# supranational/sppark

Hardware: NVIDIA H100
Metric: BLS12-381 G1 MSM/s @2^26 points (higher is better)
Workload: dtype u32x12 (384-bit Montgomery integers)

## Files before the change

### sppark_b200/build.py

```python
import os
import subprocess
import sys

HERE = os.path.dirname(os.path.abspath(__file__))
CSRC = os.path.join(HERE, "csrc")
LIB = os.environ.get("SPPARK_B200_LIB") or os.path.join(HERE, "libsppark_b200.so")

SOURCES = ["api.cu", "util/gpu.cu", "ntt/ntt.cu", "ntt/ntt_warp.cu", "poly/poly.cu", "msm/msm.cu", "msm/msm_bls12_381.cu", "msm/msm_bls12_381_g2.cu",
           "msm/msm_pasta.cu", "msm/msm_bn254_bls12_377.cu", "msm/msm_bn254_g2.cu", "msm/msm_bls12_377_g2.cu"]
NVCC_FLAGS = ["-std=c++17", "-O3", "-DSPPARK_B200_NO_WIDE_MSUB", "-gencode", "arch=compute_90a,code=sm_90a", "-lineinfo",
              "-Xcompiler", "-fPIC", "--threads", "4"]


def _sources():
    return [os.path.join(CSRC, s) for s in SOURCES if os.path.exists(os.path.join(CSRC, s))]


def _newest_input():
    newest = 0.0
    for root, _, files in os.walk(CSRC):
        for f in files:
            newest = max(newest, os.path.getmtime(os.path.join(root, f)))
    inc = os.path.join(os.path.dirname(HERE), "include", "sppark_b200.h")
    return max(newest, os.path.getmtime(inc))


def _up_to_date(obj, flags):
    dep = obj[:-2] + ".d"
    try:
        if open(obj + ".flags").read() != " ".join(flags):
            return False
        t = os.path.getmtime(obj)
        words = open(dep).read().replace("\\\n", " ").split()
        return all(os.path.getmtime(w) <= t for w in words[1:] if not w.endswith(":"))
    except OSError:
        return False


def build(force=False, verbose=False):
    if not force and os.path.exists(LIB) and os.path.getmtime(LIB) >= _newest_input():
        return LIB
    objs = []
    procs = []
    extra = os.environ.get("SPPARK_B200_NVCC_EXTRA", "").split()
    objdir = os.path.join(HERE, "build" + ("_" + os.path.basename(LIB) if extra else ""))
    os.makedirs(objdir, exist_ok=True)
    for src in _sources():
        obj = os.path.join(objdir, os.path.basename(src).replace(".cu", ".o"))
        objs.append(obj)
        if not force and not verbose and _up_to_date(obj, [*NVCC_FLAGS, *extra]):
            continue
        cmd = ["nvcc", *NVCC_FLAGS, *extra, "-MD", "-c", "-o", obj, src]
        if verbose:
            cmd.insert(1, "-Xptxas=-v")
        with open(obj + ".flags", "w") as f:
            f.write(" ".join([*NVCC_FLAGS, *extra]))
        procs.append((subprocess.Popen(cmd), cmd))
    for p, cmd in procs:
        if p.wait() != 0:
            raise RuntimeError("nvcc failed: " + " ".join(cmd))
    subprocess.check_call(["nvcc", "-shared", "-o", LIB, *objs, "-gencode", "arch=compute_90a,code=sm_90a"])
    return LIB


if __name__ == "__main__":
    print(build(force="--force" in sys.argv, verbose="-v" in sys.argv))
```

### sppark_b200/csrc/ec/xyzz.cuh

```cuda
#pragma once
#include "../ff/mont.cuh"

namespace ec {

template<class F> struct affine_t {
    F X, Y;
    HD bool is_inf() const
    {
        uint32_t acc = 0;
#pragma unroll
        for (int i = 0; i < F::N; i++) acc |= X.l[i] | Y.l[i];
        return acc == 0;
    }
};

template<class F> struct jacobian_t {
    F X, Y, Z;
};

template<class F> struct xyzz_t {
    F X, Y, ZZZ, ZZ;

    HD void set_inf()
    {
        X = F::zero(); Y = F::zero(); ZZZ = F::zero(); ZZ = F::zero();
    }
    HD bool is_inf() const
    {
        uint32_t acc = 0;
#pragma unroll
        for (int i = 0; i < F::N; i++) acc |= ZZZ.l[i] | ZZ.l[i];
        return acc == 0;
    }
    HD void set_affine(const affine_t<F>& p)
    {
        X = p.X; Y = p.Y; ZZZ = F::one(); ZZ = F::one();
    }

    HD_NOINLINE void set_double_of(const affine_t<F>& p)
    {
        F U = p.Y.dbl();
        F V = U.sqr();
        F W = U * V;
        F S = p.X * V;
        F M = p.X.sqr();
        M = M.dbl() + M;
        F X3 = M.sqr() - S - S;
        Y = M * (S - X3) - W * p.Y;
        X = X3;
        ZZ = V;
        ZZZ = W;
    }

    HD void madd(const affine_t<F>& p2)
    {
        if (p2.is_inf()) return;
        if (is_inf()) { set_affine(p2); return; }
        F P = F::mul_shared(p2.X, ZZ) - X;
        F R = F::mul_shared(p2.Y, ZZZ) - Y;
        if (P.is_zero()) {
            if (R.is_zero()) set_double_of(p2);
            else set_inf();
            return;
        }
        F PP = F::sqr_shared(P);
        F PPP = F::mul_shared(P, PP);
        F Q = F::mul_shared(X, PP);
        F X3 = F::sqr_shared(R) - PPP - Q - Q;
        Y = F::msub_shared(R, Q - X3, Y, PPP);
        X = X3;
        ZZ = F::mul_shared(ZZ, PP);
        ZZZ = F::mul_shared(ZZZ, PPP);
    }

    HD_NOINLINE void dbl()
    {
        if (is_inf()) return;
        F U = Y.dbl();
        F V = U.sqr();
        F W = U * V;
        F S = X * V;
        F M = X.sqr();
        M = M.dbl() + M;
        F X3 = M.sqr() - S - S;
        Y = M * (S - X3) - W * Y;
        X = X3;
        ZZ = ZZ * V;
        ZZZ = ZZZ * W;
    }

    HD_NOINLINE void add(const xyzz_t& p2)
    {
        if (p2.is_inf()) return;
        if (is_inf()) { *this = p2; return; }
        F U1 = X * p2.ZZ;
        F S1 = Y * p2.ZZZ;
        F P = p2.X * ZZ - U1;
        F R = p2.Y * ZZZ - S1;
        if (P.is_zero()) {
            if (R.is_zero()) dbl();
            else set_inf();
            return;
        }
        F PP = P.sqr();
        F PPP = P * PP;
        F Q = U1 * PP;
        F X3 = R.sqr() - PPP - Q - Q;
        Y = R * (Q - X3) - S1 * PPP;
        X = X3;
        ZZ = ZZ * p2.ZZ * PP;
        ZZZ = ZZZ * p2.ZZZ * PPP;
    }


    HD void dbl_hot()
    {
        if (is_inf()) return;
        F U = Y.dbl();
        F V = F::mul_shared(U, U);
        F W = F::mul_shared(U, V);
        F S = F::mul_shared(X, V);
        F M = F::mul_shared(X, X);
        M = M.dbl() + M;
        F X3 = F::mul_shared(M, M) - S - S;
        Y = F::mul_shared(M, S - X3) - F::mul_shared(W, Y);
        X = X3;
        ZZ = F::mul_shared(ZZ, V);
        ZZZ = F::mul_shared(ZZZ, W);
    }
    HD void add_hot(const xyzz_t& p2)
    {
        if (p2.is_inf()) return;
        if (is_inf()) { *this = p2; return; }
        F U1 = F::mul_shared(X, p2.ZZ);
        F S1 = F::mul_shared(Y, p2.ZZZ);
        F P = F::mul_shared(p2.X, ZZ) - U1;
        F R = F::mul_shared(p2.Y, ZZZ) - S1;
        if (P.is_zero()) {
            if (R.is_zero()) dbl_hot();
            else set_inf();
            return;
        }
        F PP = F::mul_shared(P, P);
        F PPP = F::mul_shared(P, PP);
        F Q = F::mul_shared(U1, PP);
        F X3 = F::mul_shared(R, R) - PPP - Q - Q;
        Y = F::mul_shared(R, Q - X3) - F::mul_shared(S1, PPP);
        X = X3;
        ZZ = F::mul_shared(F::mul_shared(ZZ, p2.ZZ), PP);
        ZZZ = F::mul_shared(F::mul_shared(ZZZ, p2.ZZZ), PPP);
    }

    HD jacobian_t<F> to_jacobian() const
    {
        jacobian_t<F> r;
        if (is_inf()) { r.X = F::zero(); r.Y = F::zero(); r.Z = F::zero(); return r; }
        r.X = X * ZZ;
        r.Y = Y * ZZZ;
        r.Z = ZZ;
        return r;
    }
};

}
```

### sppark_b200/csrc/ff/mont.cuh

```cuda
#pragma once
#include "../util/hd.cuh"

namespace ff {

#if defined(__CUDA_ARCH__)
namespace ptx {
DEV void mad_lo_cc(uint32_t& d, uint32_t a, uint32_t b, uint32_t c)
{   asm volatile("mad.lo.cc.u32 %0, %1, %2, %3;" : "=r"(d) : "r"(a), "r"(b), "r"(c));   }
DEV void madc_lo_cc(uint32_t& d, uint32_t a, uint32_t b, uint32_t c)
{   asm volatile("madc.lo.cc.u32 %0, %1, %2, %3;" : "=r"(d) : "r"(a), "r"(b), "r"(c));   }
DEV void madc_hi_cc(uint32_t& d, uint32_t a, uint32_t b, uint32_t c)
{   asm volatile("madc.hi.cc.u32 %0, %1, %2, %3;" : "=r"(d) : "r"(a), "r"(b), "r"(c));   }
DEV void addc(uint32_t& d, uint32_t a, uint32_t b)
{   asm volatile("addc.u32 %0, %1, %2;" : "=r"(d) : "r"(a), "r"(b));   }
DEV void add_cc(uint32_t& d, uint32_t a, uint32_t b)
{   asm volatile("add.cc.u32 %0, %1, %2;" : "=r"(d) : "r"(a), "r"(b));   }
DEV void addc_cc(uint32_t& d, uint32_t a, uint32_t b)
{   asm volatile("addc.cc.u32 %0, %1, %2;" : "=r"(d) : "r"(a), "r"(b));   }
DEV void sub_cc(uint32_t& d, uint32_t a, uint32_t b)
{   asm volatile("sub.cc.u32 %0, %1, %2;" : "=r"(d) : "r"(a), "r"(b));   }
DEV void subc_cc(uint32_t& d, uint32_t a, uint32_t b)
{   asm volatile("subc.cc.u32 %0, %1, %2;" : "=r"(d) : "r"(a), "r"(b));   }
DEV void subc(uint32_t& d, uint32_t a, uint32_t b)
{   asm volatile("subc.u32 %0, %1, %2;" : "=r"(d) : "r"(a), "r"(b));   }
}
#endif

template<class C>
struct mont_t {
    static constexpr int N = C::N;
    uint32_t l[N];

    static HD mont_t zero()
    {
        mont_t r;
#pragma unroll
        for (int i = 0; i < N; i++) r.l[i] = 0;
        return r;
    }
    static HD mont_t one()
    {
        mont_t r;
#pragma unroll
        for (int i = 0; i < N; i++) r.l[i] = C::ONE(i);
        return r;
    }
    static HD mont_t rr()
    {
        mont_t r;
#pragma unroll
        for (int i = 0; i < N; i++) r.l[i] = C::RR(i);
        return r;
    }
    HD bool is_zero() const
    {
        uint32_t acc = 0;
#pragma unroll
        for (int i = 0; i < N; i++) acc |= l[i];
        return acc == 0;
    }
    friend HD bool operator==(const mont_t& a, const mont_t& b)
    {
        uint32_t acc = 0;
#pragma unroll
        for (int i = 0; i < N; i++) acc |= a.l[i] ^ b.l[i];
        return acc == 0;
    }

    static HD mont_t final_sub(const mont_t& a, uint32_t top_carry = 0)
    {
        mont_t r;
#if defined(__CUDA_ARCH__)
        uint32_t t[N], borrow;
        ptx::sub_cc(t[0], a.l[0], C::P(0));
#pragma unroll
        for (int i = 1; i < N; i++) ptx::subc_cc(t[i], a.l[i], C::P(i));
        ptx::subc(borrow, top_carry, 0);
#pragma unroll
        for (int i = 0; i < N; i++) r.l[i] = borrow ? a.l[i] : t[i];
#else
        uint32_t t[N];
        int64_t br = 0;
        for (int i = 0; i < N; i++) {
            int64_t d = (int64_t)a.l[i] - C::P(i) + br;
            t[i] = (uint32_t)d;
            br = d >> 32;
        }
        br += top_carry;
        for (int i = 0; i < N; i++) r.l[i] = br < 0 ? a.l[i] : t[i];
#endif
        return r;
    }

    friend HD mont_t operator+(const mont_t& a, const mont_t& b)
    {
        mont_t s;
        uint32_t carry;
#if defined(__CUDA_ARCH__)
        ptx::add_cc(s.l[0], a.l[0], b.l[0]);
#pragma unroll
        for (int i = 1; i < N; i++) ptx::addc_cc(s.l[i], a.l[i], b.l[i]);
        ptx::addc(carry, 0, 0);
#else
        uint64_t c = 0;
        for (int i = 0; i < N; i++) {
            c += (uint64_t)a.l[i] + b.l[i];
            s.l[i] = (uint32_t)c;
            c >>= 32;
        }
        carry = (uint32_t)c;
#endif
        return final_sub(s, carry);
    }

    friend HD mont_t operator-(const mont_t& a, const mont_t& b)
    {
        mont_t d;
#if defined(__CUDA_ARCH__)
        uint32_t borrow;
        ptx::sub_cc(d.l[0], a.l[0], b.l[0]);
#pragma unroll
        for (int i = 1; i < N; i++) ptx::subc_cc(d.l[i], a.l[i], b.l[i]);
        ptx::subc(borrow, 0, 0);
        ptx::add_cc(d.l[0], d.l[0], C::P(0) & borrow);
#pragma unroll
        for (int i = 1; i < N - 1; i++) ptx::addc_cc(d.l[i], d.l[i], C::P(i) & borrow);
        ptx::addc(d.l[N - 1], d.l[N - 1], C::P(N - 1) & borrow);
#else
        int64_t br = 0;
        for (int i = 0; i < N; i++) {
            int64_t x = (int64_t)a.l[i] - b.l[i] + br;
            d.l[i] = (uint32_t)x;
            br = x >> 32;
        }
        if (br) {
            uint64_t c = 0;
            for (int i = 0; i < N; i++) {
                c += (uint64_t)d.l[i] + C::P(i);
                d.l[i] = (uint32_t)c;
                c >>= 32;
            }
        }
#endif
        return d;
    }

    HD mont_t neg() const { return is_zero() ? *this : zero() - *this; }
    HD mont_t cneg(bool flag) const { return flag ? neg() : *this; }
    HD mont_t dbl() const { return *this + *this; }

#if defined(__CUDA_ARCH__)
    template<int I, class V>
    static DEV void row(uint32_t (&E)[2 * N + 2], uint32_t (&O)[2 * N + 2], uint32_t x, const V& v)
    {
        constexpr bool even_row = (I & 1) == 0;
        uint32_t (&A1)[2 * N + 2] = even_row ? E : O;
        uint32_t (&A2)[2 * N + 2] = even_row ? O : E;
        ptx::mad_lo_cc(A1[I], x, v[0], A1[I]);
        ptx::madc_hi_cc(A1[I + 1], x, v[0], A1[I + 1]);
#pragma unroll
        for (int j = 2; j < N; j += 2) {
            ptx::madc_lo_cc(A1[I + j], x, v[j], A1[I + j]);
            ptx::madc_hi_cc(A1[I + j + 1], x, v[j], A1[I + j + 1]);
        }
        ptx::addc(A1[I + N], A1[I + N], 0);
        ptx::mad_lo_cc(A2[I + 1], x, v[1], A2[I + 1]);
        ptx::madc_hi_cc(A2[I + 2], x, v[1], A2[I + 2]);
#pragma unroll
        for (int j = 3; j < N; j += 2) {
            ptx::madc_lo_cc(A2[I + j], x, v[j], A2[I + j]);
            ptx::madc_hi_cc(A2[I + j + 1], x, v[j], A2[I + j + 1]);
        }
        ptx::addc(A2[I + N + 1], A2[I + N + 1], 0);
    }

    struct modulus_view {
        DEV uint32_t operator[](int j) const { return C::P(j); }
    };

    template<int I>
    static DEV void rows(uint32_t (&E)[2 * N + 2], uint32_t (&O)[2 * N + 2], uint32_t& c,
                         const mont_t& a, const mont_t& b)
    {
        if constexpr (I < N) {
            row<I>(E, O, a.l[I], b.l);
            uint32_t m = (E[I] + O[I] + c) * C::M0;
            row<I>(E, O, m, modulus_view());
            uint64_t s = (uint64_t)E[I] + O[I] + c;
            c = (uint32_t)(s >> 32);
            rows<I + 1>(E, O, c, a, b);
        }
    }
#endif

    friend HD mont_t operator*(const mont_t& a, const mont_t& b) { return mul_inline(a, b); }

#if defined(__CUDA_ARCH__)
    struct wide_t { uint32_t l[2 * N]; };

    template<int I, int W, class V>
    static DEV void row_w(uint32_t* E, uint32_t* O, uint32_t x, const V& v)
    {
        uint32_t* A1 = (I & 1) == 0 ? E : O;
        uint32_t* A2 = (I & 1) == 0 ? O : E;
        ptx::mad_lo_cc(A1[I], x, v[0], A1[I]);
        ptx::madc_hi_cc(A1[I + 1], x, v[0], A1[I + 1]);
#pragma unroll
        for (int j = 2; j < W; j += 2) {
            ptx::madc_lo_cc(A1[I + j], x, v[j], A1[I + j]);
            ptx::madc_hi_cc(A1[I + j + 1], x, v[j], A1[I + j + 1]);
        }
        ptx::addc(A1[I + W + (W & 1)], A1[I + W + (W & 1)], 0);
        ptx::mad_lo_cc(A2[I + 1], x, v[1], A2[I + 1]);
        ptx::madc_hi_cc(A2[I + 2], x, v[1], A2[I + 2]);
#pragma unroll
        for (int j = 3; j < W; j += 2) {
            ptx::madc_lo_cc(A2[I + j], x, v[j], A2[I + j]);
            ptx::madc_hi_cc(A2[I + j + 1], x, v[j], A2[I + j + 1]);
        }
        ptx::addc(A2[I + W + 1 - (W & 1)], A2[I + W + 1 - (W & 1)], 0);
    }
    template<int I, int W>
    static DEV void mul_rows_w(uint32_t* E, uint32_t* O, const uint32_t* a, const uint32_t* b)
    {
        if constexpr (I < W) {
            row_w<I, W>(E, O, a[I], b);
            mul_rows_w<I + 1, W>(E, O, a, b);
        }
    }
    template<int W>
    static DEV void mul_wide_w(uint32_t* t, const uint32_t* a, const uint32_t* b)
    {
        uint32_t E[2 * W + 2], O[2 * W + 2];
#pragma unroll
        for (int i = 0; i < 2 * W + 2; i++) E[i] = O[i] = 0;
        mul_rows_w<0, W>(E, O, a, b);
        ptx::add_cc(t[0], E[0], O[0]);
#pragma unroll
        for (int i = 1; i < 2 * W - 1; i++) ptx::addc_cc(t[i], E[i], O[i]);
        ptx::addc(t[2 * W - 1], E[2 * W - 1], O[2 * W - 1]);
    }

    template<int W>
    static DEV uint32_t abs_diff_w(uint32_t* d, const uint32_t* x, const uint32_t* y)
    {
        uint32_t borrow;
        ptx::sub_cc(d[0], x[0], y[0]);
#pragma unroll
        for (int i = 1; i < W; i++) ptx::subc_cc(d[i], x[i], y[i]);
        ptx::subc(borrow, 0, 0);
        ptx::sub_cc(d[0], d[0] ^ borrow, borrow);
#pragma unroll
        for (int i = 1; i < W - 1; i++) ptx::subc_cc(d[i], d[i] ^ borrow, borrow);
        ptx::subc(d[W - 1], d[W - 1] ^ borrow, borrow);
        return borrow & 1;
    }

    static DEV wide_t mul_wide(const mont_t& a, const mont_t& b)
    {
        wide_t t;
#if defined(SPPARK_B200_KARATSUBA)
        constexpr bool karatsuba = N % 4 == 0 && N >= 8;
#else
        constexpr bool karatsuba = false;
#endif
        if constexpr (karatsuba) {
            constexpr int H = N / 2;
            uint32_t da[H], db[H], zm[2 * H], z0h[H], top, cf;
            const uint32_t neg = 0u - (abs_diff_w<H>(da, a.l, a.l + H) ^ abs_diff_w<H>(db, b.l + H, b.l));
            mul_wide_w<H>(t.l, a.l, b.l);
            mul_wide_w<H>(t.l + 2 * H, a.l + H, b.l + H);
            mul_wide_w<H>(zm, da, db);
#pragma unroll
            for (int i = 0; i < H; i++) z0h[i] = t.l[H + i];
            ptx::add_cc(t.l[H], t.l[H], t.l[2 * H]);
#pragma unroll
            for (int i = 1; i < 2 * H; i++) ptx::addc_cc(t.l[H + i], t.l[H + i], t.l[2 * H + i]);
            ptx::addc(top, 0, 0);
            ptx::add_cc(t.l[H], t.l[H], t.l[0]);
#pragma unroll
            for (int i = 1; i < H; i++) ptx::addc_cc(t.l[H + i], t.l[H + i], t.l[i]);
#pragma unroll
            for (int i = 0; i < H; i++) ptx::addc_cc(t.l[2 * H + i], t.l[2 * H + i], z0h[i]);
            ptx::addc(top, top, 0);
            ptx::add_cc(cf, neg, neg);
#pragma unroll
            for (int i = 0; i < 2 * H; i++) ptx::addc_cc(t.l[H + i], t.l[H + i], zm[i] ^ neg);
            ptx::addc(top, top, neg);
            ptx::add_cc(t.l[3 * H], t.l[3 * H], top);
#pragma unroll
            for (int i = 3 * H + 1; i < 2 * N - 1; i++) ptx::addc_cc(t.l[i], t.l[i], 0);
            ptx::addc(t.l[2 * N - 1], t.l[2 * N - 1], 0);
        } else {
            mul_wide_w<N>(t.l, a.l, b.l);
        }
        return t;
    }

    template<int I>
    static DEV void sqr_rows(uint32_t* E, uint32_t* O, uint32_t& c, const uint32_t* a, const uint32_t* d)
    {
        if constexpr (I < N) {
            if constexpr (I < N - 1) {
                uint32_t v[N - I];
                v[0] = a[I];
                v[1] = a[I + 1] << 1;
#pragma unroll
                for (int k = 2; k < N - I; k++) v[k] = d[I + k];
                row_w<2 * I, N - I>(E, O, a[I], v);
            } else {
                ptx::mad_lo_cc(E[2 * I], a[I], a[I], E[2 * I]);
                ptx::madc_hi_cc(E[2 * I + 1], a[I], a[I], E[2 * I + 1]);
                ptx::addc(E[2 * I + 2], E[2 * I + 2], 0);
            }
            uint32_t m = (E[I] + O[I] + c) * C::M0;
            row_w<I, N>(E, O, m, modulus_view());
            uint64_t s = (uint64_t)E[I] + O[I] + c;
            c = (uint32_t)(s >> 32);
            sqr_rows<I + 1>(E, O, c, a, d);
        }
    }
    static DEV mont_t sqr_inline(const mont_t& a)
    {
        if constexpr (C::P(N - 1) >= 0x55555555u) {
            return mul_inline(a, a);
        } else {
            uint32_t E[2 * N + 2], O[2 * N + 2], d[N], c = 0;
#pragma unroll
            for (int i = 0; i < 2 * N + 2; i++) E[i] = O[i] = 0;
#pragma unroll
            for (int j = 1; j < N; j++) d[j] = __funnelshift_l(a.l[j - 1], a.l[j], 1);
            sqr_rows<0>(E, O, c, a.l, d);
            mont_t r;
            ptx::add_cc(r.l[0], E[N], c);
#pragma unroll
            for (int i = 1; i < N; i++) ptx::addc_cc(r.l[i], E[N + i], 0);
            ptx::add_cc(r.l[0], r.l[0], O[N]);
#pragma unroll
            for (int i = 1; i < N - 1; i++) ptx::addc_cc(r.l[i], r.l[i], O[N + i]);
            ptx::addc(r.l[N - 1], r.l[N - 1], O[2 * N - 1]);
            return final_sub(r);
        }
    }

    static DEV wide_t sub_wide(const wide_t& x, const wide_t& y)
    {
        wide_t t;
        ptx::sub_cc(t.l[0], x.l[0], y.l[0]);
#pragma unroll
        for (int i = 1; i < 2 * N - 1; i++) ptx::subc_cc(t.l[i], x.l[i], y.l[i]);
        ptx::subc(t.l[2 * N - 1], x.l[2 * N - 1], y.l[2 * N - 1]);
        ptx::add_cc(t.l[N], t.l[N], C::P(0));
#pragma unroll
        for (int i = 1; i < N - 1; i++) ptx::addc_cc(t.l[N + i], t.l[N + i], C::P(i));
        ptx::addc(t.l[2 * N - 1], t.l[2 * N - 1], C::P(N - 1));
        return t;
    }

    template<int I>
    static DEV void redc_rows(uint32_t* E, uint32_t* O, uint32_t& c, const wide_t& t)
    {
        if constexpr (I < N) {
            uint32_t m = (t.l[I] + E[I] + O[I] + c) * C::M0;
            row_w<I, N>(E, O, m, modulus_view());
            uint64_t s = (uint64_t)t.l[I] + E[I] + O[I] + c;
            c = (uint32_t)(s >> 32);
            redc_rows<I + 1>(E, O, c, t);
        }
    }
    template<int K>
    static DEV mont_t redc(const wide_t& t)
    {
        uint32_t E[2 * N + 2], O[2 * N + 2], c = 0;
#pragma unroll
        for (int i = 0; i < 2 * N + 2; i++) E[i] = O[i] = 0;
        redc_rows<0>(E, O, c, t);
        mont_t r;
        uint32_t top, k;
        ptx::add_cc(r.l[0], t.l[N], c);
#pragma unroll
        for (int i = 1; i < N; i++) ptx::addc_cc(r.l[i], t.l[N + i], 0);
        ptx::addc(top, 0, 0);
        ptx::add_cc(r.l[0], r.l[0], E[N]);
#pragma unroll
        for (int i = 1; i < N; i++) ptx::addc_cc(r.l[i], r.l[i], E[N + i]);
        ptx::addc(k, 0, 0);
        top += k;
        ptx::add_cc(r.l[0], r.l[0], O[N]);
#pragma unroll
        for (int i = 1; i < N; i++) ptx::addc_cc(r.l[i], r.l[i], O[N + i]);
        ptx::addc(k, 0, 0);
        top += k;
        r = final_sub(r, top);
        if constexpr (K > 1) r = final_sub(r);
        return r;
    }

    static __device__ __noinline__ mont_t mul_shared(mont_t a, mont_t b)
    {
#if defined(SPPARK_B200_KARATSUBA)
        return redc<1>(mul_wide(a, b));
#else
        return mul_inline(a, b);
#endif
    }
    static __device__ __noinline__ mont_t sqr_shared(mont_t a) { return sqr_inline(a); }
    static __device__ __noinline__ mont_t msub_shared(mont_t a, mont_t b, mont_t c, mont_t d)
    {
#if defined(SPPARK_B200_NO_WIDE_MSUB)
        return mul_inline(a, b) - mul_inline(c, d);
#else
        return redc<2>(sub_wide(mul_wide(a, b), mul_wide(c, d)));
#endif
    }
#else
    static inline mont_t mul_shared(const mont_t& a, const mont_t& b) { return mul_inline(a, b); }
    static inline mont_t sqr_shared(const mont_t& a) { return mul_inline(a, a); }
    static inline mont_t msub_shared(const mont_t& a, const mont_t& b, const mont_t& c, const mont_t& d)
    {   return mul_inline(a, b) - mul_inline(c, d);   }
#endif

    static HD mont_t mul_inline(const mont_t& a, const mont_t& b)
    {
        mont_t r;
#if defined(__CUDA_ARCH__)
        uint32_t E[2 * N + 2], O[2 * N + 2], c = 0;
#pragma unroll
        for (int i = 0; i < 2 * N + 2; i++) E[i] = O[i] = 0;
        rows<0>(E, O, c, a, b);
        ptx::add_cc(r.l[0], E[N], c);
#pragma unroll
        for (int i = 1; i < N; i++) ptx::addc_cc(r.l[i], E[N + i], 0);
        ptx::add_cc(r.l[0], r.l[0], O[N]);
#pragma unroll
        for (int i = 1; i < N - 1; i++) ptx::addc_cc(r.l[i], r.l[i], O[N + i]);
        ptx::addc(r.l[N - 1], r.l[N - 1], O[2 * N - 1]);
#else
        uint32_t t[N + 2];
        for (int i = 0; i < N + 2; i++) t[i] = 0;
        for (int i = 0; i < N; i++) {
            uint64_t c = 0;
            for (int j = 0; j < N; j++) {
                c += (uint64_t)a.l[j] * b.l[i] + t[j];
                t[j] = (uint32_t)c;
                c >>= 32;
            }
            c += t[N];
            t[N] = (uint32_t)c;
            t[N + 1] = (uint32_t)(c >> 32);
            uint32_t m = t[0] * C::M0;
            c = ((uint64_t)m * C::P(0) + t[0]) >> 32;
            for (int j = 1; j < N; j++) {
                c += (uint64_t)m * C::P(j) + t[j];
                t[j - 1] = (uint32_t)c;
                c >>= 32;
            }
            c += t[N];
            t[N - 1] = (uint32_t)c;
            t[N] = t[N + 1] + (uint32_t)(c >> 32);
        }
        for (int i = 0; i < N; i++) r.l[i] = t[i];
        return final_sub(r, t[N]);
#endif
        return final_sub(r);
    }

    HD mont_t sqr() const { return *this * *this; }

    HD mont_t to_mont() const { return *this * rr(); }
    HD mont_t from_mont() const
    {
        mont_t o = zero();
        o.l[0] = 1;
        return *this * o;
    }
    HD mont_t inv() const
    {
        mont_t acc = one(), base = *this;
        uint32_t e[N];
        uint32_t borrow = 2;
        for (int i = 0; i < N; i++) {
            uint32_t pi = C::P(i);
            e[i] = pi - borrow;
            borrow = pi < borrow ? 1 : 0;
        }
        for (int i = N * 32 - 1; i >= 0; i--) {
            acc = acc.sqr();
            if ((e[i / 32] >> (i % 32)) & 1) acc = acc * base;
        }
        return acc;
    }
};

}
```

### sppark_b200/csrc/msm/msm_bls12_381.cu

```cuda
#include "msm_host.cuh"

RustError msm_host_bls12_381(void* out, const void* points, size_t npoints, const void* scalars,
                             size_t stride, bool has_flag, bool mont)
{
    return msm_host<ff::bls12_381_fp_t>(out, points, npoints, scalars, stride, has_flag,
                                        mont ? scalars_from_mont<ff::bls12_381_fr_t> : nullptr);
}
RustError msm_dev_bls12_381(void* out, const void* d_points, size_t npoints, const void* d_scalars, void* stream)
{   return msm_dev<ff::bls12_381_fp_t>(out, d_points, npoints, d_scalars, stream);   }

RustError gen_points_bls12_381(void* d_out, size_t n, void* stream)
{   return gen_points_dev<ff::bls12_381_g1_gen>(d_out, n, stream);   }
RustError combine_bls12_381(void* out, const void* partials, size_t count)
{   return combine_host<ff::bls12_381_fp_t>(out, partials, count);   }

extern "C" RustError mult_pippenger(void* out, const void* points, size_t npoints, const void* scalars)
{   return msm_host_bls12_381(out, points, npoints, scalars, 96, false, false);   }

extern "C" RustError mult_pippenger_inf(void* out, const void* points, size_t npoints,
                                        const void* scalars, size_t ffi_affine_sz)
{   return msm_host_bls12_381(out, points, npoints, scalars, ffi_affine_sz, true, false);   }

template<class F>
__global__ void selftest_kernel(int op, size_t n, uint32_t* r, const uint32_t* a, const uint32_t* b)
{
    size_t i = blockIdx.x * (size_t)blockDim.x + threadIdx.x;
    if (i >= n) return;
    F x, y, z;
    for (int k = 0; k < F::N; k++) { x.l[k] = a[i * F::N + k]; y.l[k] = b[i * F::N + k]; }
    switch (op) {
    case 0: z = x * y; break;
    case 1: z = x + y; break;
    case 2: z = x - y; break;
    case 3: z = x.sqr(); break;
    case 4: z = F::mul_shared(x, y); break;
    case 5: z = F::sqr_shared(x); break;
    default: z = F::msub_shared(x, y, y, x.sqr()); break;
    }
    for (int k = 0; k < F::N; k++) r[i * F::N + k] = z.l[k];
}

template<class F>
static RustError selftest(int op, size_t n, void* r, const void* a, const void* b)
{
    try {
        const gpu_t& gpu = select_gpu(-1);
        const stream_t& s = gpu[0];
        size_t bytes = n * F::N * 4;
        dev_ptr_t<uint32_t> da(n * F::N, s), db(n * F::N, s), dr(n * F::N, s);
        s.HtoD(da, a, bytes);
        s.HtoD(db, b, bytes);
        selftest_kernel<F><<<(unsigned)((n + 127) / 128), 128, 0, s>>>(op, n, dr, da, db);
        COUNT_LAUNCH();
        CUDA_OK(cudaGetLastError());
        s.DtoH(r, dr, bytes);
        s.sync();
    } catch (const cuda_error& e) {
        return rust_err(e.code(), e.what());
    }
    return rust_ok();
}

extern "C" RustError sppark_b200_selftest_field(int field, int op, size_t n, void* r, const void* a, const void* b)
{
    switch (field) {
    case 0: return selftest<ff::bls12_381_fp_t>(op, n, r, a, b);
    case 1: return selftest<ff::bls12_381_fr_t>(op, n, r, a, b);
    case 2: return selftest<ff::pallas_fp_t>(op, n, r, a, b);
    case 3: return selftest<ff::vesta_fp_t>(op, n, r, a, b);
    case 4: return selftest<ff::bn254_fp_t>(op, n, r, a, b);
    case 5: return selftest<ff::bn254_fr_t>(op, n, r, a, b);
    case 6: return selftest<ff::bls12_377_fp_t>(op, n, r, a, b);
    case 7: return selftest<ff::bls12_377_fr_t>(op, n, r, a, b);
    default: return rust_err(-(int)cudaErrorInvalidValue, "selftest: unknown field");
    }
}

RustError msm_preload_bls12_381(const void* points, size_t npoints, size_t stride, bool has_flag, void** d_points,
                                uint32_t* copies, uint32_t* wbits)
{   return msm_preload<ff::bls12_381_fp_t>(points, npoints, stride, has_flag, d_points, copies, wbits);   }
RustError msm_resident_bls12_381(void* out, const void* d_points, size_t npoints, const void* scalars, bool mont,
                                 uint32_t wbits, uint32_t copies, size_t stride)
{
    return msm_resident<ff::bls12_381_fp_t, ff::bls12_381_fr_t>(out, d_points, npoints, scalars, mont, wbits, copies, stride);
}

extern "C" RustError sppark_b200_selftest_msm_sort(size_t n, uint32_t wbits, uint32_t cap, const void* scalars,
                                                   void* counts, void* offsets, void* sorted, void* heavy_slots,
                                                   uint32_t* info)
{
    using namespace msm;
    if (n == 0 || n >= (1ull << 31) || wbits < 3 || wbits > 24 || cap > SORT_CAP)
        return rust_err(-(int)cudaErrorInvalidValue, "selftest_msm_sort: bad arguments");
    try {
        const gpu_t& gpu = select_gpu(-1);
        const stream_t& s = gpu[0];
        Config cfg = make_config(n);
        cfg.wbits = wbits;
        cfg.nwins = (256 + wbits - 1) / wbits;
        cfg.lg_nb = wbits - 1;
        const size_t nslots = (size_t)cfg.nwins << cfg.lg_nb, entries = (size_t)cfg.nwins * n;
        const size_t nbins = (size_t)cfg.nwins << sort_lg_bins(cfg, n);
        const size_t heavy_cap = entries / (cfg.heavy + 1) + 1, chunk_cap = entries / cfg.heavy_chunk + heavy_cap;
        dev_ptr_t<uint32_t> d_sc(8 * n, s), d_counts(nslots, s), d_offsets(nslots, s), d_cursor(nslots, s);
        dev_ptr_t<uint32_t> d_ctrl(4, s), d_heavy(3 * heavy_cap, s), d_cmap(chunk_cap, s), d_sorted(entries, s);
        dev_ptr_t<uint32_t> d_bcount(nbins, s), d_bbase(nbins, s), d_bcur(nbins, s), d_over(nbins, s);
        dev_ptr_t<uint32_t> d_staging(2 * entries, s);
        s.HtoD(d_sc, scalars, 32 * n);
        const SortBufs sb{d_counts, d_offsets, d_cursor, d_ctrl, d_heavy, d_cmap, d_sorted,
                          d_bcount, d_bbase, d_bcur, d_over, reinterpret_cast<uint2*>((uint32_t*)d_staging)};
        sort_slice(cfg, cap ? cap : SORT_CAP, d_sc, sb, (uint32_t)gpu.sm_count(), s);
        uint32_t ctrl[4];
        s.DtoH(ctrl, d_ctrl, 16);
        s.DtoH(counts, d_counts, nslots * 4);
        s.DtoH(offsets, d_offsets, nslots * 4);
        s.DtoH(sorted, d_sorted, entries * 4);
        s.sync();
        std::vector<uint32_t> hl(3 * (size_t)ctrl[1] + 1);
        if (ctrl[1]) s.DtoH(hl.data(), d_heavy, 12 * (size_t)ctrl[1]);
        s.sync();
        for (uint32_t h = 0; h < ctrl[1]; h++) static_cast<uint32_t*>(heavy_slots)[h] = hl[3 * h];
        info[0] = cfg.nwins; info[1] = cfg.heavy; info[2] = ctrl[1]; info[3] = sort_lg_bins(cfg, n); info[4] = ctrl[3];
    } catch (const cuda_error& e) {
        return rust_err(e.code(), e.what());
    }
    return rust_ok();
}
```

### sppark_b200/msm.py

```python
import numpy as np

from . import _lib

BLS12_381_G1, PALLAS, VESTA, BLS12_381_G2, BN254_G1, BLS12_377_G1, BN254_G2, BLS12_377_G2 = 0, 1, 2, 3, 4, 5, 6, 7
_LIMBS = {BLS12_381_G1: 6, PALLAS: 4, VESTA: 4, BLS12_381_G2: 12, BN254_G1: 4, BLS12_377_G1: 6, BN254_G2: 8, BLS12_377_G2: 12}


def _check(points, scalars):
    if points.shape[0] != scalars.shape[0]:
        raise ValueError("length mismatch")
    if not (points.flags["C_CONTIGUOUS"] and scalars.flags["C_CONTIGUOUS"]):
        raise TypeError("points and scalars must be C-contiguous")
    if points.dtype != np.uint64 or scalars.dtype != np.uint64 or scalars.shape[1] != 4:
        raise TypeError("points/scalars must be uint64 limb arrays")


def multi_scalar_mult(points, scalars):
    _check(points, scalars)
    assert points.shape[1] == 12
    out = np.zeros(18, dtype=np.uint64)
    err = _lib.lib().mult_pippenger(out.ctypes.data, points.ctypes.data, points.shape[0], scalars.ctypes.data)
    _lib.check(err)
    return out


def multi_scalar_mult_arkworks(points, scalars):
    _check(points, scalars)
    assert points.shape[1] == 13
    out = np.zeros(18, dtype=np.uint64)
    err = _lib.lib().mult_pippenger_inf(out.ctypes.data, points.ctypes.data, points.shape[0],
                                        scalars.ctypes.data, points.strides[0])
    _lib.check(err)
    return out


def multi_scalar_mult_fp2_arkworks(points, scalars):
    _check(points, scalars)
    assert points.shape[1] == 25
    out = np.zeros(36, dtype=np.uint64)
    err = _lib.lib().mult_pippenger_fp2_inf(out.ctypes.data, points.ctypes.data, points.shape[0],
                                            scalars.ctypes.data, points.strides[0])
    _lib.check(err)
    return out


def msm(curve, points, scalars, mont=False):
    _check(points, scalars)
    nl = _LIMBS[curve]
    assert points.shape[1] in (2 * nl, 2 * nl + 1)
    out = np.zeros(3 * nl, dtype=np.uint64)
    err = _lib.lib().sppark_b200_msm_ex(curve, out.ctypes.data, points.ctypes.data, points.shape[0],
                                        scalars.ctypes.data, points.strides[0], int(mont))
    _lib.check(err)
    return out


class MsmContext:

    def __init__(self, curve, points, precompute=None):
        import ctypes as C
        if points.dtype != np.uint64 or not points.flags["C_CONTIGUOUS"]:
            raise TypeError("points must be a C-contiguous uint64 limb array")
        nl = _LIMBS[curve]
        assert points.shape[1] in (2 * nl, 2 * nl + 1)
        self.curve, self.npoints, self._h = curve, points.shape[0], C.c_void_p()
        if precompute is None:
            err = _lib.lib().sppark_b200_msm_ctx_create(curve, points.ctypes.data, points.shape[0],
                                                        points.strides[0], C.byref(self._h))
        else:
            err = _lib.lib().sppark_b200_msm_ctx_create_precomputed(curve, points.ctypes.data, points.shape[0],
                                                                    points.strides[0], int(precompute),
                                                                    C.byref(self._h))
        _lib.check(err)

    def invoke(self, scalars, mont=False):
        if scalars.dtype != np.uint64 or scalars.ndim != 2 or scalars.shape[1] != 4 or not scalars.flags["C_CONTIGUOUS"]:
            raise TypeError("scalars must be a C-contiguous (n, 4) uint64 array")
        out = np.zeros(3 * _LIMBS[self.curve], dtype=np.uint64)
        _lib.check(_lib.lib().sppark_b200_msm_ctx_invoke(self._h, out.ctypes.data, scalars.ctypes.data,
                                                         scalars.shape[0], int(mont)))
        return out

    def close(self):
        if self._h:
            _lib.lib().sppark_b200_msm_ctx_free(self._h)
            self._h = None

    def __del__(self):
        try:
            self.close()
        except Exception:
            pass


def msm_dev(curve, d_points, d_scalars, npoints=None, stream=None):
    import torch
    nl = _LIMBS[curve]
    assert d_points.is_cuda and d_scalars.is_cuda and d_points.is_contiguous() and d_scalars.is_contiguous()
    n = npoints if npoints is not None else d_scalars.numel() * d_scalars.element_size() // 32
    out = np.zeros(3 * nl, dtype=np.uint64)
    with torch.cuda.device(d_points.device):
        s = stream if stream is not None else torch.cuda.current_stream().cuda_stream
        err = _lib.lib().sppark_b200_msm_dev(curve, out.ctypes.data, d_points.data_ptr(), n,
                                             d_scalars.data_ptr(), s)
    _lib.check(err)
    return out


def generate_points_dev(curve, n, device=None):
    import torch
    nl = _LIMBS[curve]
    out = torch.empty((n, 2 * nl), dtype=torch.int64, device=device or "cuda")
    with torch.cuda.device(out.device):
        err = _lib.lib().sppark_b200_generate_points_dev(curve, out.data_ptr(), n,
                                                         torch.cuda.current_stream().cuda_stream)
    _lib.check(err)
    return out


def combine(curve, partials):
    partials = np.ascontiguousarray(partials, dtype=np.uint64)
    out = np.zeros(3 * _LIMBS[curve], dtype=np.uint64)
    _lib.check(_lib.lib().sppark_b200_msm_combine(curve, out.ctypes.data, partials.ctypes.data, partials.shape[0]))
    return out


def selftest_field(field, op, a, b):
    a = np.ascontiguousarray(a, dtype=np.uint64)
    b = np.ascontiguousarray(b, dtype=np.uint64)
    r = np.zeros_like(a)
    err = _lib.lib().sppark_b200_selftest_field(field, {"mul": 0, "add": 1, "sub": 2, "sqr": 3, "mul_shared": 4, "sqr_shared": 5, "msub_shared": 6}[op],
                                                a.shape[0], r.ctypes.data, a.ctypes.data, b.ctypes.data)
    _lib.check(err)
    return r
```

Before: 2.411.

## Fuse a*b - c*d into one interleaved Montgomery reduction and use squarings in hot EC ops

Replaces the wide-product msub (and the two-separate-multiplications fallback) with a fused Montgomery routine. It computes a*b + c*(p-d) row by row with a single interleaved reduction, so only one final subtraction is needed. The compile flag that disabled wide msub is removed, so the new path is always used. The hot doubling and addition formulas now call dedicated squaring and msub helpers instead of generic multiplies, which cuts multiplication and reduction work per bucket operation. A selftest op is added to validate the fused routine; the fused accumulator relies on modulus headroom and adds register pressure.

Result: faster. 2.565, median of 6 (+6.4%).

```diff
diff --git a/sppark_b200/build.py b/sppark_b200/build.py
--- a/sppark_b200/build.py
+++ b/sppark_b200/build.py
@@ -8,7 +8,7 @@
 
 SOURCES = ["api.cu", "util/gpu.cu", "ntt/ntt.cu", "ntt/ntt_warp.cu", "poly/poly.cu", "msm/msm.cu", "msm/msm_bls12_381.cu", "msm/msm_bls12_381_g2.cu",
            "msm/msm_pasta.cu", "msm/msm_bn254_bls12_377.cu", "msm/msm_bn254_g2.cu", "msm/msm_bls12_377_g2.cu"]
-NVCC_FLAGS = ["-std=c++17", "-O3", "-DSPPARK_B200_NO_WIDE_MSUB", "-gencode", "arch=compute_90a,code=sm_90a", "-lineinfo",
+NVCC_FLAGS = ["-std=c++17", "-O3", "-gencode", "arch=compute_90a,code=sm_90a", "-lineinfo",
               "-Xcompiler", "-fPIC", "--threads", "4"]
 
 
diff --git a/sppark_b200/csrc/ec/xyzz.cuh b/sppark_b200/csrc/ec/xyzz.cuh
--- a/sppark_b200/csrc/ec/xyzz.cuh
+++ b/sppark_b200/csrc/ec/xyzz.cuh
@@ -117,13 +117,13 @@
     {
         if (is_inf()) return;
         F U = Y.dbl();
-        F V = F::mul_shared(U, U);
+        F V = F::sqr_shared(U);
         F W = F::mul_shared(U, V);
         F S = F::mul_shared(X, V);
-        F M = F::mul_shared(X, X);
+        F M = F::sqr_shared(X);
         M = M.dbl() + M;
-        F X3 = F::mul_shared(M, M) - S - S;
-        Y = F::mul_shared(M, S - X3) - F::mul_shared(W, Y);
+        F X3 = F::sqr_shared(M) - S - S;
+        Y = F::msub_shared(M, S - X3, W, Y);
         X = X3;
         ZZ = F::mul_shared(ZZ, V);
         ZZZ = F::mul_shared(ZZZ, W);
@@ -141,11 +141,11 @@
             else set_inf();
             return;
         }
-        F PP = F::mul_shared(P, P);
+        F PP = F::sqr_shared(P);
         F PPP = F::mul_shared(P, PP);
         F Q = F::mul_shared(U1, PP);
-        F X3 = F::mul_shared(R, R) - PPP - Q - Q;
-        Y = F::mul_shared(R, Q - X3) - F::mul_shared(S1, PPP);
+        F X3 = F::sqr_shared(R) - PPP - Q - Q;
+        Y = F::msub_shared(R, Q - X3, S1, PPP);
         X = X3;
         ZZ = F::mul_shared(F::mul_shared(ZZ, p2.ZZ), PP);
         ZZZ = F::mul_shared(F::mul_shared(ZZZ, p2.ZZZ), PPP);
diff --git a/sppark_b200/csrc/ff/mont.cuh b/sppark_b200/csrc/ff/mont.cuh
--- a/sppark_b200/csrc/ff/mont.cuh
+++ b/sppark_b200/csrc/ff/mont.cuh
@@ -191,6 +191,21 @@
             rows<I + 1>(E, O, c, a, b);
         }
     }
+
+    template<int I>
+    static DEV void msub_rows(uint32_t (&E)[2 * N + 2], uint32_t (&O)[2 * N + 2], uint32_t& k,
+                              const mont_t& a, const mont_t& b, const mont_t& c, const mont_t& dn)
+    {
+        if constexpr (I < N) {
+            row<I>(E, O, a.l[I], b.l);
+            row<I>(E, O, c.l[I], dn.l);
+            uint32_t m = (E[I] + O[I] + k) * C::M0;
+            row<I>(E, O, m, modulus_view());
+            uint64_t s = (uint64_t)E[I] + O[I] + k;
+            k = (uint32_t)(s >> 32);
+            msub_rows<I + 1>(E, O, k, a, b, c, dn);
+        }
+    }
 #endif
 
     friend HD mont_t operator*(const mont_t& a, const mont_t& b) { return mul_inline(a, b); }
@@ -343,18 +358,30 @@
         }
     }
 
-    static DEV wide_t sub_wide(const wide_t& x, const wide_t& y)
-    {
-        wide_t t;
-        ptx::sub_cc(t.l[0], x.l[0], y.l[0]);
-#pragma unroll
-        for (int i = 1; i < 2 * N - 1; i++) ptx::subc_cc(t.l[i], x.l[i], y.l[i]);
-        ptx::subc(t.l[2 * N - 1], x.l[2 * N - 1], y.l[2 * N - 1]);
-        ptx::add_cc(t.l[N], t.l[N], C::P(0));
-#pragma unroll
-        for (int i = 1; i < N - 1; i++) ptx::addc_cc(t.l[N + i], t.l[N + i], C::P(i));
-        ptx::addc(t.l[2 * N - 1], t.l[2 * N - 1], C::P(N - 1));
-        return t;
+    static DEV mont_t msub_inline(const mont_t& a, const mont_t& b, const mont_t& c, const mont_t& d)
+    {
+        if constexpr (C::P(N - 1) >= 0x55555555u) {
+            return mul_inline(a, b) - mul_inline(c, d);
+        } else {
+            mont_t dn;
+            ptx::sub_cc(dn.l[0], C::P(0), d.l[0]);
+#pragma unroll
+            for (int i = 1; i < N - 1; i++) ptx::subc_cc(dn.l[i], C::P(i), d.l[i]);
+            ptx::subc(dn.l[N - 1], C::P(N - 1), d.l[N - 1]);
+            uint32_t E[2 * N + 2], O[2 * N + 2], k = 0;
+#pragma unroll
+            for (int i = 0; i < 2 * N + 2; i++) E[i] = O[i] = 0;
+            msub_rows<0>(E, O, k, a, b, c, dn);
+            mont_t r;
+            ptx::add_cc(r.l[0], E[N], k);
+#pragma unroll
+            for (int i = 1; i < N; i++) ptx::addc_cc(r.l[i], E[N + i], 0);
+            ptx::add_cc(r.l[0], r.l[0], O[N]);
+#pragma unroll
+            for (int i = 1; i < N - 1; i++) ptx::addc_cc(r.l[i], r.l[i], O[N + i]);
+            ptx::addc(r.l[N - 1], r.l[N - 1], O[2 * N - 1]);
+            return final_sub(r);
+        }
     }
 
     template<int I>
@@ -406,13 +433,7 @@
     }
     static __device__ __noinline__ mont_t sqr_shared(mont_t a) { return sqr_inline(a); }
     static __device__ __noinline__ mont_t msub_shared(mont_t a, mont_t b, mont_t c, mont_t d)
-    {
-#if defined(SPPARK_B200_NO_WIDE_MSUB)
-        return mul_inline(a, b) - mul_inline(c, d);
-#else
-        return redc<2>(sub_wide(mul_wide(a, b), mul_wide(c, d)));
-#endif
-    }
+    {   return msub_inline(a, b, c, d);   }
 #else
     static inline mont_t mul_shared(const mont_t& a, const mont_t& b) { return mul_inline(a, b); }
     static inline mont_t sqr_shared(const mont_t& a) { return mul_inline(a, a); }
diff --git a/sppark_b200/csrc/msm/msm_bls12_381.cu b/sppark_b200/csrc/msm/msm_bls12_381.cu
--- a/sppark_b200/csrc/msm/msm_bls12_381.cu
+++ b/sppark_b200/csrc/msm/msm_bls12_381.cu
@@ -27,6 +27,16 @@
     size_t i = blockIdx.x * (size_t)blockDim.x + threadIdx.x;
     if (i >= n) return;
     F x, y, z;
+    if (op == 7) {
+        F c, d;
+        for (int k = 0; k < F::N; k++) {
+            x.l[k] = a[2 * i * F::N + k]; c.l[k] = a[(2 * i + 1) * F::N + k];
+            y.l[k] = b[2 * i * F::N + k]; d.l[k] = b[(2 * i + 1) * F::N + k];
+        }
+        z = F::msub_shared(x, y, c, d);
+        for (int k = 0; k < F::N; k++) r[i * F::N + k] = z.l[k];
+        return;
+    }
     for (int k = 0; k < F::N; k++) { x.l[k] = a[i * F::N + k]; y.l[k] = b[i * F::N + k]; }
     switch (op) {
     case 0: z = x * y; break;
@@ -46,10 +56,10 @@
     try {
         const gpu_t& gpu = select_gpu(-1);
         const stream_t& s = gpu[0];
-        size_t bytes = n * F::N * 4;
-        dev_ptr_t<uint32_t> da(n * F::N, s), db(n * F::N, s), dr(n * F::N, s);
-        s.HtoD(da, a, bytes);
-        s.HtoD(db, b, bytes);
+        const size_t bytes = n * F::N * 4, in_bytes = op == 7 ? 2 * bytes : bytes;
+        dev_ptr_t<uint32_t> da(in_bytes / 4, s), db(in_bytes / 4, s), dr(n * F::N, s);
+        s.HtoD(da, a, in_bytes);
+        s.HtoD(db, b, in_bytes);
         selftest_kernel<F><<<(unsigned)((n + 127) / 128), 128, 0, s>>>(op, n, dr, da, db);
         COUNT_LAUNCH();
         CUDA_OK(cudaGetLastError());
diff --git a/sppark_b200/msm.py b/sppark_b200/msm.py
--- a/sppark_b200/msm.py
+++ b/sppark_b200/msm.py
@@ -128,8 +128,11 @@
 def selftest_field(field, op, a, b):
     a = np.ascontiguousarray(a, dtype=np.uint64)
     b = np.ascontiguousarray(b, dtype=np.uint64)
-    r = np.zeros_like(a)
-    err = _lib.lib().sppark_b200_selftest_field(field, {"mul": 0, "add": 1, "sub": 2, "sqr": 3, "mul_shared": 4, "sqr_shared": 5, "msub_shared": 6}[op],
-                                                a.shape[0], r.ctypes.data, a.ctypes.data, b.ctypes.data)
+    if a.shape != b.shape or (op == "msub4" and a.shape[0] % 2):
+        raise ValueError("selftest_field: operand shapes")
+    n = a.shape[0] // 2 if op == "msub4" else a.shape[0]
+    r = np.zeros((n, a.shape[1]), dtype=np.uint64)
+    ops = {"mul": 0, "add": 1, "sub": 2, "sqr": 3, "mul_shared": 4, "sqr_shared": 5, "msub_shared": 6, "msub4": 7}
+    err = _lib.lib().sppark_b200_selftest_field(field, ops[op], n, r.ctypes.data, a.ctypes.data, b.ctypes.data)
     _lib.check(err)
     return r
```
